# probsys/AutoGP.jl

Hardware: AMD Instinct MI355X
Metric: particle_logpdf_evals_per_sec (higher is better)
Workload: dtype f64

## Files before the change

### autogp.jl_amd/csrc/agp_chol_kernel.hpp

```cpp
#pragma once
#include <type_traits>
#include "agp_common.hpp"
#include "agp_cov_kernel.hpp"

namespace agp {

__device__ __forceinline__ double readlane_d(double v, int lane) {
  int lo = __double2loint(v), hi = __double2hiint(v);
  lo = __builtin_amdgcn_readlane(lo, lane);
  hi = __builtin_amdgcn_readlane(hi, lane);
  return __hiloint2double(hi, lo);
}

__device__ __forceinline__ d4 mfma(double a, double b, d4 c) {
  return __builtin_amdgcn_mfma_f64_16x16x4f64(a, b, c, 0, 0, 0);
}

__device__ __forceinline__ int blk_idx(int rb, int cb) { return rb * (rb + 1) / 2 + cb; }
__device__ __forceinline__ int tri_idx(int i, int j) { return i * (i + 1) / 2 + j; }

__device__ __forceinline__ void mfma_prio_on() { __builtin_amdgcn_s_setprio(1); }
__device__ __forceinline__ void mfma_prio_off() { __builtin_amdgcn_s_setprio(0); }
__device__ __forceinline__ int sblk_idx(int jb, int lb) { return jb * (jb - 1) / 2 + lb; }

// ... 139 lines not shown
    if (jb == 0) AGP_DPROBE(5);

    {
      const int nrem = NSB - 1 - jb;
      const int npair = nrem * (nrem + 1) / 2;
      auto upd = [&](int ib, int cb, bool on, d4& x) {
        (void)on;
        const double* blk = sm + blk_idx(ib, cb) * 256;
#pragma unroll
        for (int r = 0; r < 4; ++r) x[r] = blk[64 * r + l];
      };
      if (w == 0) {
        if (npair > 0) {
          double* blk = sm + blk_idx(jb + 1, jb + 1) * 256;
          const double* la = sm + blk_idx(jb + 1, jb) * 256;
          d4 x;
          double f[4];
#pragma unroll
          for (int r = 0; r < 4; ++r) { x[r] = blk[64 * r + l]; f[r] = la[64 * r + l]; }
#pragma unroll
          for (int s4 = 0; s4 < 4; ++s4) x = mfma(-f[s4], f[s4], x);
#pragma unroll
          for (int r = 0; r < 4; ++r) blk[64 * r + l] = x[r];
        }
      } else {
        int e = w, ii = 1, cc = w - 1;
        if (cc > ii) { cc -= ii + 1; ++ii; }
        auto advance = [&](int& e_, int& ii_, int& cc_) {
          e_ += 3; cc_ += 3;
          while (cc_ > ii_) { cc_ -= ii_ + 1; ++ii_; }
        };
        while (e < npair) {
          int eb[3], ib3[3], cb3[3];
#pragma unroll
          for (int u = 0; u < 3; ++u) {
            eb[u] = e; ib3[u] = jb + 1 + ii; cb3[u] = jb + 1 + cc;
            advance(e, ii, cc);
          }
          d4 x[3];
          double fa[3][4], fb[3][4];
#pragma unroll
          for (int u = 0; u < 3; ++u) {
            const bool on = eb[u] < npair;
            const int ib = on ? ib3[u] : jb + 1, cb = on ? cb3[u] : jb + 1;
            upd(ib, cb, on, x[u]);
            const double* la = sm + blk_idx(cb, jb) * 256;
            const double* lb = sm + blk_idx(ib, jb) * 256;
#pragma unroll
            for (int s4 = 0; s4 < 4; ++s4) { fa[u][s4] = -la[64 * s4 + l]; fb[u][s4] = lb[64 * s4 + l]; }
          }
#pragma unroll
          for (int s4 = 0; s4 < 4; ++s4)
#pragma unroll
            for (int u = 0; u < 3; ++u) x[u] = mfma(fa[u][s4], fb[u][s4], x[u]);
#pragma unroll
          for (int u = 0; u < 3; ++u)
            if (eb[u] < npair) {
              double* blk = sm + blk_idx(ib3[u], cb3[u]) * 256;
#pragma unroll
              for (int r = 0; r < 4; ++r) blk[64 * r + l] = x[u][r];
            }
        }
      }
      if (tid >= NB && tid - NB >= (jb + 1) * 16) {
        const int ti_ = tid - NB;
        const double* lb = sm + blk_idx(ti_ >> 4, jb) * 256;
        double t0 = rvec[ti_], t1 = 0.0;
#pragma unroll
        for (int q = 0; q < 16; q += 2) {
          t0 = fma(-lb[q * 16 + (ti_ & 15)], avec[jb * 16 + q], t0);
          t1 = fma(-lb[(q + 1) * 16 + (ti_ & 15)], avec[jb * 16 + q + 1], t1);
        }
        rvec[ti_] = t0 + t1;
      }
      if (jb == 0) AGP_DPROBE(6);
      if (w == 0 && jb + 1 < nbk) factor16(jb + 1);
      if (jb == 0) AGP_DPROBE(7);
    }
    __syncthreads();
    if (jb == 0) AGP_DPROBE(8);
  }
  if (nbk < NSB) {
    for (int jb = nbk + w; jb < NSB; jb += 4) {
      double* Wg = a.W + (((long long)p * a.wsteps + a.k % a.wsteps) * NSB + jb) * 256;
#pragma unroll
      for (int r = 0; r < 4; ++r) Wg[l15 * 16 + 4 * r + lq] = (l15 == 4 * r + lq) ? 1.0 : 0.0;
    }
    if (tid >= nbk * 16 && tid < NB) avec[tid] = 0.0;
    __syncthreads();
  }
  AGP_DPROBE(9);

  if (mark && tid == 0) *mark = (long long)wall_clock64();
  for (int bi = 0; bi < NSB * NSB / 2; ++bi) {
    const int rb = 2 * (bi >> 3) + ((tid >> 3) & 1), cb = bi & 7;
    const int c = tid >> 4, r2 = 2 * (tid & 7);
    if (rb >= cb)
      *reinterpret_cast<d2*>(Tt + (cb * 16 + c) * NB + rb * 16 + r2) = *reinterpret_cast<const d2*>(sm + blk_idx(rb, cb) * 256 + c * 16 + r2);
  }
  AGP_DPROBE(10);
  if (tid < NB) {
    vecp[tk * NB + tid] = avec[tid];
    const double dii = sm[blk_idx(tid >> 4, tid >> 4) * 256 + 17 * (tid & 15)];
    Wl[tid] = 2.0 * log(dii);
  }
  __syncthreads();
  if (w == 0) {
    double ss = avec[l] * avec[l] + avec[l + 64] * avec[l + 64];
    double ld = Wl[l] + Wl[l + 64];
#pragma unroll
    for (int off = 32; off > 0; off >>= 1) { ss += __shfl_xor(ss, off); ld += __shfl_xor(ld, off); }
    if (l == 0) {
      double* pp = a.partial + ((long long)p * (a.ntp ? a.ntp : a.nt) + tk) * 2;
      pp[0] = ld;
      pp[1] = ss;
      if (bad != 0 && a.info[p] == 0) a.info[p] = bad;
    }
  }
  if (INTRSM) {
    asm volatile("s_waitcnt vmcnt(0)" ::: "memory");
    __syncthreads();
    if (tid == 0) {
      __builtin_amdgcn_fence(__ATOMIC_RELEASE, "agent");
      asm volatile("s_waitcnt vmcnt(0)" ::: "memory");
      __hip_atomic_store(a.ready + p, a.k + 1, __ATOMIC_RELAXED, __HIP_MEMORY_SCOPE_AGENT);
      if (a.tflag != nullptr) __hip_atomic_store(a.tflag + (long long)p * a.ntri + tri_idx(tk, tk), 1, __ATOMIC_RELAXED, __HIP_MEMORY_SCOPE_AGENT);
    }
  }
  AGP_DPROBE(11);
}

__device__ __forceinline__ d2 ld_pair(const double* T, int col, int rowA) {
  return *reinterpret_cast<const d2*>(T + col * NB + rowA);
}
__device__ __forceinline__ void st_pair(double* T, int col, int rowA, double a0, double a1) {
  d2 v; v.x = a0; v.y = a1;
  *reinterpret_cast<d2*>(T + col * NB + rowA) = v;
}

struct FlowProbe { double wait; long long ph[4]; };
#ifdef AGP_EXPERIMENTS
#define AGP_TRACE(a) ((a).trace)
#else
#define AGP_TRACE(a) (static_cast<long long*>(nullptr))
#endif
#define AGP_PROBE(i) do { if (AGP_TRACE(a) && wait_acc && tid == 0) wait_acc->ph[i] = (long long)wall_clock64(); } while (0)
typedef int v4i_t __attribute__((ext_vector_type(4)));
__device__ __forceinline__ __amdgpu_buffer_rsrc_t tile_row_rsrc(const double* base) {
  return __builtin_amdgcn_make_buffer_rsrc(const_cast<double*>(base), 0, 0x7fffffff, 0x00020000);
}
__device__ __forceinline__ d2 buf_load_d2(__amdgpu_buffer_rsrc_t r, unsigned voff_bytes, int soff_bytes) {
  return __builtin_bit_cast(d2, __builtin_amdgcn_raw_buffer_load_b128(r, voff_bytes, soff_bytes, 0));
}
__device__ __forceinline__ bool flow_wait(const int* flag) {
  int spins = 0;
  while (__hip_atomic_load(flag, __ATOMIC_RELAXED, __HIP_MEMORY_SCOPE_AGENT) == 0) {
    __builtin_amdgcn_s_sleep(1);
    if (++spins > (1 << 24)) return false;
  }
  return true;
}
template <bool FACTOR, int DCOV, bool INTRSM, int DM, int GM, bool FLOW>
__device__ __forceinline__ void chol_tile(const CholArgs& a, const int p_, const int ps_, const int ti_, const int tk_,
                                          const int jmax_, const bool is_diag, double* sm, const int tid,
                                          FlowProbe* wait_acc = nullptr) {
  constexpr bool TAB = GM == 1, LAGM = GM == 2;
  const int p = __builtin_amdgcn_readfirstlane(p_), ps = __builtin_amdgcn_readfirstlane(ps_);
  const int ti = __builtin_amdgcn_readfirstlane(ti_), tk = __builtin_amdgcn_readfirstlane(tk_);
  const int jmax = __builtin_amdgcn_readfirstlane(jmax_);
  double* rvec = sm + U_MAIN_DOUBLES;
  double* avec = rvec + 128;
  double* xv = avec + 128;
  double* Wl = xv + 64;
  (void)p;
  const int l = tid & 63;
  const int w = tid >> 6;
  const int l15 = l & 15, lq = l >> 4;
  const int row0 = 32 * w + 2 * l15;
  const int row1 = row0 + 1;

  double* __restrict__ Ap = a.A + (long long)ps * a.strideA;
  double* vecp = a.vec + (long long)ps * a.ldv;

  double* __restrict__ Tt = Ap + tile_off(ti, tk);
  d4 acc[NSB][2];
  const bool prebuilt = (DCOV == 0) || (p >= a.n_fused);
  auto run_eval = [&]() {
    const ProgHdr h = a.hdr[p];
    double* tpt = sm;
    double* sig = sm + 256;
    const double* lagt = sig + h.n_cp * 256;
    const bool rankt = LAGM && a.lagr != nullptr;
    const int lstride = rankt ? a.lag_stride : 256;
    int* xrk = reinterpret_cast<int*>(sig + h.n_cp * 256 + (LAGM ? h.n_lag * lstride : 0));
    const int* rk = rankt ? xrk : nullptr;
    const bool cltm = rankt && a.clt.B != nullptr;
    int* cbl = xrk + 256;
    const int* cbp = cltm ? cbl - (a.clt.W > 0 && ti > tk ? (ti - tk) * NB - (NB - 1) : 0) : nullptr;
    double* prm = reinterpret_cast<double*>(xrk) + (rankt ? 128 + (cltm ? a.clt.nB / 2 : 0) : 0);
    int* ops = reinterpret_cast<int*>(prm + h.n_prm + 2);
    for (int i = tid; i < h.n_prm + 2; i += 256) prm[i] = a.prm[h.prm_off + i];
    for (int i = tid; i < h.n_ops; i += 256) ops[i] = (int)a.ops[h.op_off + i];
    double* etab = sm + U_MAIN_DOUBLES;
    if (AGP_EXP_TABLE && !LAGM && tid < AGP_EXP_TAB_N) etab[tid] = fm::c_exp_tab[tid];
    cov_prologue<LAGM>(a.tt, a.code, ti, tk, h, ops, prm, tpt, sig, tid, a.lagtab, a.nt, LAGM ? a.lagr : nullptr, lstride, xrk, true, a.clt, cbl);
    const double noise = !FACTOR ? 0.0 : DM == 2 ? a.noise[p] : diag_noise(a.noise, a.noise_q, p, tk, a.n1_pad);
    const bool use_tab = TAB && (h.flags & 1) != 0;
    const double* __restrict__ ltile = a.logdt + tile_off(ti, tk);
    double ltn[4] = {0.0, 0.0, 0.0, 0.0};
    auto fetch_lt = [&](int t) {
      const int cbn = t >> 1, rsn = (t & 1) ? row1 : row0;
#pragma unroll
      for (int r = 0; r < 4; ++r) ltn[r] = ltile[(cbn * 16 + 4 * r + lq) * NB + rsn];
    };
    if (use_tab) fetch_lt(0);
    const bool one_node = h.n_ops == 1;
    const int op1 = one_node ? __builtin_amdgcn_readfirstlane(ops[0]) : -1;
    const double q0 = one_node ? prm[0] : 0.0, q1 = one_node ? prm[1] : 0.0, q2 = one_node ? prm[2] : 0.0;
    const bool pure_lag = LAGM && one_node && op1 == OP_LAG && ti != tk && (ti + 1) * NB <= a.n1 && (tk + 1) * NB <= a.n1;
    if (pure_lag) {
      const double* lq_ = lagt + (NB - 1);
      const int rk0 = rk ? rk[row0] : 0, rk1 = rk ? rk[row1] : 0;
#pragma unroll
      for (int cb = 0; cb < NSB; ++cb)
#pragma unroll
        for (int r = 0; r < 4; ++r) {
          const int cs = cb * 16 + 4 * r + lq;
          double v0, v1;
          if (cbp) {
            const int rc = rk[NB + cs], e0 = rk0 - rc, e1 = rk1 - rc, d0 = e0 < 0 ? -e0 : e0, d1 = e1 < 0 ? -e1 : e1;
            v0 = -lagt[(d0 & CLT_MASK) + cbp[d0 >> CLT_SHIFT]]; v1 = -lagt[(d1 & CLT_MASK) + cbp[d1 >> CLT_SHIFT]];
          } else if (rk) {
            const int rc = rk[NB + cs], d0 = rk0 - rc, d1 = rk1 - rc;
            v0 = -lagt[d0 < 0 ? -d0 : d0]; v1 = -lagt[d1 < 0 ? -d1 : d1];
          } else {
            v0 = -lq_[row0 - cs]; v1 = -lq_[row1 - cs];
          }
          acc[cb][0][r] = v0; acc[cb][1][r] = v1;
        }
    }
    const bool pure_lin = one_node && op1 == OP_LIN && ti != tk && (ti + 1) * NB <= a.n1 && (tk + 1) * NB <= a.n1;
    if (pure_lin) {
      const double u0 = tpt[row0] - q0, u1 = tpt[row1] - q0;
#pragma unroll
      for (int cb = 0; cb < NSB; ++cb)
#pragma unroll
        for (int r = 0; r < 4; ++r) {
          const double tcc = tpt[NB + cb * 16 + 4 * r + lq] - q0;
          const double v0 = -(q1 + q2 * (u0 * tcc)), v1 = -(q1 + q2 * (u1 * tcc));
          acc[cb][0][r] = v0; acc[cb][1][r] = v1;
        }
    }
#pragma unroll 1
    for (int t = (pure_lag || pure_lin) ? 16 : 0; t < 16; ++t) {
      const int cb = t >> 1, st = t & 1;
      const int rslot = st ? row1 : row0;
      double tr[4], tc[4], out[4];
      double lt[4];
      int ri[4], ci[4];
#pragma unroll
      for (int r = 0; r < 4; ++r) lt[r] = ltn[r];
      if (use_tab && t + 1 < 16) fetch_lt(t + 1);
#pragma unroll
      for (int r = 0; r < 4; ++r) {
        const int cslot = cb * 16 + 4 * r + lq;
        tr[r] = tpt[rslot]; tc[r] = tpt[NB + cslot];
        ri[r] = rslot; ci[r] = NB + cslot;
      }
      if (one_node) {
        eval_leaf<4, (LAGM ? 3 : TAB ? 2 : 1)>(op1, q0, q1, q2, sig, lagt, tr, tc, ri, ci, lt, etab, out, rk, cbp);
      } else {
        eval_program<(DCOV > 0 ? DCOV : 4), 4, (LAGM ? 3 : TAB ? 2 : 1)>(h, ops, prm, sig, tr, tc, ri, ci, lt, out, etab, lagt, rk, lstride, cbp);
      }
      d4 v;
#pragma unroll
      for (int r = 0; r < 4; ++r)
        v[r] = -cov_finalize(out[r], ti * NB + rslot, tk * NB + cb * 16 + 4 * r + lq, a.n1, a.n1_pad, a.m2, noise);
      auto put = [&](d4& dst) { dst = v; };
      switch (t) {
        case 0: put(acc[0][0]); break;  case 1: put(acc[0][1]); break;  case 2: put(acc[1][0]); break;  case 3: put(acc[1][1]); break;
        case 4: put(acc[2][0]); break;  case 5: put(acc[2][1]); break;  case 6: put(acc[3][0]); break;  case 7: put(acc[3][1]); break;
        case 8: put(acc[4][0]); break;  case 9: put(acc[4][1]); break;  case 10: put(acc[5][0]); break; case 11: put(acc[5][1]); break;
        case 12: put(acc[6][0]); break; case 13: put(acc[6][1]); break; case 14: put(acc[7][0]); break; default: put(acc[7][1]); break;
      }
    }
    __syncthreads();
  };
  if (!prebuilt) {
    run_eval();
  } else {
#pragma unroll
    for (int cb = 0; cb < NSB; ++cb) { acc[cb][0] = d4{0.0, 0.0, 0.0, 0.0}; acc[cb][1] = d4{0.0, 0.0, 0.0, 0.0}; }
  }

  double rv = 0.0;
  if (is_diag && tid < NB) rv = vecp[tk * NB + tid];
  if (FLOW) AGP_PROBE(0);

  constexpr int KS = KB;
  constexpr int NU = KS / 4;
  constexpr int SLABS_PER_TILE = NB / KS;
  constexpr int SLAB_DOUBLES = KS * LDS_STRIDE;
  static_assert(4 * SLAB_DOUBLES <= U_MAIN_DOUBLES, "slab buffers");
  const int jfirst = FACTOR ? 0 : a.j0;
  const int nslab = (jmax - jfirst) * SLABS_PER_TILE;
  if (nslab > 0) {
    const int scol0 = tid >> 6;
    const int srow = 2 * (tid & 63);
    const unsigned offB = (unsigned)(scol0 * NB + srow);
    const unsigned offA = (unsigned)(lq * NB + row0);
    double rx = 0.0;
    const __amdgpu_buffer_rsrc_t rsA = tile_row_rsrc(Ap + tile_off(ti, 0)), rsB = tile_row_rsrc(Ap + tile_off(tk, 0));
    auto gload = [&](int s, d2 (&ra_)[NU], d2 (&rb_)[NU]) {
      const int sb = (jfirst * SLABS_PER_TILE + s) * (KS * NB * 8);
#pragma unroll
      for (int u = 0; u < NU; ++u) {
        ra_[u] = buf_load_d2(rsA, offA * 8, sb + u * (4 * NB * 8));
        rb_[u] = buf_load_d2(rsB, offB * 8, sb + u * (4 * NB * 8));
      }
      if (is_diag && tid < KS) rx = vecp[(jfirst * SLABS_PER_TILE + s) * KS + tid];
    };
    auto lstore = [&](int buf, const d2 (&ra_)[NU], const d2 (&rb_)[NU]) {
      double* Bs = sm + buf * SLAB_DOUBLES;
#pragma unroll
      for (int u = 0; u < NU; ++u) {
        *reinterpret_cast<d2*>(Bs + (scol0 + 4 * u) * LDS_STRIDE + srow) = rb_[u];
      }
      if (is_diag && tid < KS) xv[buf * KS + tid] = rx;
    };

    auto flow_ready = [&](int j) {
      const long long tw0 = AGP_TRACE(a) ? (long long)wall_clock64() : 0;
      const int* tf = a.tflag + (long long)ps * a.ntri;
      bool ok = flow_wait(tf + tri_idx(tk, j));
      if (!is_diag) ok = flow_wait(tf + tri_idx(ti, j)) && ok;
      if (!ok) a.info[ps] = -7;
      __builtin_amdgcn_fence(__ATOMIC_ACQUIRE, "agent");
      if (AGP_TRACE(a) && wait_acc) wait_acc->wait += (double)((long long)wall_clock64() - tw0);
    };
    int all_ready = 0;
    if (FLOW) {
      int probe = 0;
      if (tid == 0) {
        const int* tf = a.tflag + (long long)ps * a.ntri;
        const int jl = jfirst + (nslab - 1) / SLABS_PER_TILE;
        probe = __hip_atomic_load(tf + tri_idx(tk, jl), __ATOMIC_RELAXED, __HIP_MEMORY_SCOPE_AGENT) != 0 &&
                (is_diag || __hip_atomic_load(tf + tri_idx(ti, jl), __ATOMIC_RELAXED, __HIP_MEMORY_SCOPE_AGENT) != 0);
        if (probe) __builtin_amdgcn_fence(__ATOMIC_ACQUIRE, "agent");
        else flow_ready(jfirst);
      }
      all_ready = __syncthreads_or(probe);
    }
    d2 fx[NU], fy[NU], rb[NU];
    gload(0, fx, rb);
    lstore(0, fx, rb);
    __syncthreads();
    auto slab = [&](const int s, const int buf, const d2 (&fr)[NU], d2 (&rn)[NU], auto last) {
      constexpr bool LAST = decltype(last)::value;
      if constexpr (!LAST) gload(s + 1, rn, rb);
      const double* Bs = sm + buf * SLAB_DOUBLES;
      mfma_prio_on();
#pragma unroll
      for (int kk = 0; kk < KS / 4; ++kk) {
        const int krow = (kk * 4 + lq) * LDS_STRIDE;
        double fa[NSB];
#pragma unroll
        for (int cb = 0; cb < NSB; ++cb) fa[cb] = Bs[krow + cb * 16 + l15];
        d2 fb;
        fb = fr[kk];
#pragma unroll
        for (int cb = 0; cb < NSB; ++cb) {
          acc[cb][0] = mfma(fa[cb], fb.x, acc[cb][0]);
          acc[cb][1] = mfma(fa[cb], fb.y, acc[cb][1]);
        }
      }
      mfma_prio_off();
      if (is_diag && tid < NB) {
        const double* xs_ = xv + buf * KS;
#pragma unroll
        for (int kk = 0; kk < KS; ++kk) rv = fma(-Bs[kk * LDS_STRIDE + tid], xs_[kk], rv);
      }
      if constexpr (!LAST) lstore(buf ^ 1, rn, rb);
      if (FLOW && !all_ready && tid == 0 && s + 2 < nslab && (s + 2) % SLABS_PER_TILE == 0) flow_ready(jfirst + (s + 2) / SLABS_PER_TILE);
      __syncthreads();
    };
    constexpr std::false_type more{};
    int s = 0;
    for (; s + 2 < nslab; s += 2) {
      slab(s, 0, fx, fy, more);
      slab(s + 1, 1, fy, fx, more);
    }
    slab(s, 0, fx, fy, more);
    slab(s + 1, 1, fy, fx, std::true_type{});
  }

  if (FLOW) AGP_PROBE(1);
  if (prebuilt) {
#pragma unroll
    for (int cb = 0; cb < NSB; ++cb) {
#pragma unroll
      for (int r = 0; r < 4; ++r) {
        const d2 t2 = ld_pair(Tt, cb * 16 + 4 * r + lq, row0);
        acc[cb][0][r] -= t2.x;
        acc[cb][1][r] -= t2.y;
      }
      __builtin_amdgcn_sched_barrier(0);
    }
  }

  if (!FACTOR || (!is_diag && !INTRSM)) {
#pragma unroll
    for (int cb = 0; cb < NSB; ++cb) {
#pragma unroll
      for (int r = 0; r < 4; ++r) {
        st_pair(Tt, cb * 16 + 4 * r + lq, row0, -acc[cb][0][r], -acc[cb][1][r]);
      }
      __builtin_amdgcn_sched_barrier(0);
    }
    if (is_diag && tid < NB) vecp[tk * NB + tid] = rv;
    return;
  }

  if (!is_diag) {
    if (tid == 0) {
      if (FLOW) {
        const long long tw0 = AGP_TRACE(a) ? (long long)wall_clock64() : 0;
        if (!flow_wait(a.tflag + (long long)ps * a.ntri + tri_idx(tk, tk))) a.info[ps] = -7;
        if (AGP_TRACE(a) && wait_acc) wait_acc->wait += (double)((long long)wall_clock64() - tw0);
      } else {
        const int want = a.k + 1;
        int spins = 0;
        while (__hip_atomic_load(a.ready + ps, __ATOMIC_RELAXED, __HIP_MEMORY_SCOPE_AGENT) < want) {
          __builtin_amdgcn_s_sleep(8);
          if (++spins > (1 << 22)) { a.info[ps] = -7; break; }
        }
      }
      __builtin_amdgcn_fence(__ATOMIC_ACQUIRE, "agent");
    }
    __syncthreads();
    {
      const double* __restrict__ Lkk = Ap + tile_off(a.k, a.k);
      const double* __restrict__ Wg = a.W + ((long long)ps * a.wsteps + a.k % a.wsteps) * NSB * 256;
      const int c = tid >> 4, r = tid & 15;
#pragma unroll
      for (int jb = 1; jb < NSB; ++jb)
#pragma unroll
        for (int lb = 0; lb < jb; ++lb)
          sm[sblk_idx(jb, lb) * 256 + tid] = Lkk[(lb * 16 + c) * NB + jb * 16 + r];
#pragma unroll
      for (int u = 0; u < NSB; ++u) sm[(T_NBLK + u) * 256 + tid] = -Wg[u * 256 + tid];
    }
    __syncthreads();
    if (FLOW) AGP_PROBE(2);
#pragma unroll
    for (int jb = 0; jb < NSB; ++jb) {
#pragma unroll
      for (int lb = 0; lb < jb; ++lb) {
        const double* blk = sm + sblk_idx(jb, lb) * 256;
#pragma unroll
        for (int s4 = 0; s4 < 4; ++s4) {
          const double fl = blk[64 * s4 + l];
          acc[jb][0] = mfma(fl, acc[lb][0][s4], acc[jb][0]);
          acc[jb][1] = mfma(fl, acc[lb][1][s4], acc[jb][1]);
        }
      }
      d4 x0 = d4{0.0, 0.0, 0.0, 0.0}, x1 = d4{0.0, 0.0, 0.0, 0.0};
#pragma unroll
      for (int s4 = 0; s4 < 4; ++s4) {
        const double fw = sm[(T_NBLK + jb) * 256 + 64 * s4 + l];
        x0 = mfma(fw, acc[jb][0][s4], x0);
        x1 = mfma(fw, acc[jb][1][s4], x1);
      }
      acc[jb][0] = x0;
      acc[jb][1] = x1;
#pragma unroll
      for (int r = 0; r < 4; ++r) {
        st_pair(Tt, jb * 16 + 4 * r + lq, row0, x0[r], x1[r]);
      }
    }
    if (FLOW) {
      AGP_PROBE(3);
      asm volatile("s_waitcnt vmcnt(0)" ::: "memory");
      __syncthreads();
      if (tid == 0) {
        __builtin_amdgcn_fence(__ATOMIC_RELEASE, "agent");
        asm volatile("s_waitcnt vmcnt(0)" ::: "memory");
        __hip_atomic_store(a.tflag + (long long)ps * a.ntri + tri_idx(ti, tk), 1, __ATOMIC_RELAXED, __HIP_MEMORY_SCOPE_AGENT);
      }
    }
    return;
  }

#pragma unroll
  for (int st = 0; st < 2; ++st) {
    const int rw = st ? row1 : row0;
    const int rb = rw >> 4, rr = rw & 15;
#pragma unroll
    for (int cb = 0; cb < NSB; ++cb)
      if (rb >= cb) {
        double* blk = sm + blk_idx(rb, cb) * 256;
#pragma unroll
        for (int r = 0; r < 4; ++r) blk[(4 * r + lq) * 16 + rr] = -acc[cb][st][r];
      }
  }
  factor_diag_tile<INTRSM>(a, ps, tk, Tt, vecp, sm, rvec, avec, Wl, rv, tid);
}

template <bool FACTOR, int DCOV, bool INTRSM, int DM = 0, int GM = 0>
__global__ __launch_bounds__(256, 2) void k_chol_update(CholArgs a) {
  static_assert(GM == 0 || DCOV > 0, "the log|dt| table / the lag tables only matter to instantiations that evaluate tiles");
  static_assert(DM == 0 || (FACTOR && INTRSM), "split launches exist for the in-kernel-solve factorisation only");
  static_assert(DM == 0 || DM == 2, "the diagonal-only launch is k_chol_diag");
  __shared__ __attribute__((aligned(16))) double sm[U_MAIN_DOUBLES + U_EXTRA_DOUBLES];

  int b = blockIdx.x;
  int xcd, qq;
  int T, ti, tk, jmax;
  int pl, tl;
  if (DM == 2) {
    T = a.tiles;
    xcd = b & 7; qq = b >> 3;
    pl = qq / T; tl = a.t0 + (qq - pl * T);
    tk = a.k; ti = a.k + tl; jmax = a.k;
  } else if (FACTOR) {
    T = a.tiles;
    const int ndiag = 8 * ((a.P + 7) / 8);
    if (b < ndiag) {
      xcd = b & 7; pl = b >> 3; tl = 0;
    } else {
      b -= ndiag;
      xcd = b & 7; qq = b >> 3;
      pl = qq / (T - 1); tl = 1 + (qq - pl * (T - 1));
    }
    tk = a.k; ti = a.k + tl; jmax = a.rl ? 0 : a.k;
  } else {
    xcd = b & 7; qq = b >> 3;
    const int nt2 = a.nt - a.nt1;
    if (a.schur_diag_only) {
      T = nt2;
      pl = qq / T; tl = qq - pl * T;
      ti = tk = a.nt1 + tl; jmax = a.nt1;
    } else {
      T = nt2 * (nt2 + 1) / 2;
      pl = qq / T; tl = qq - pl * T;
      int ii = (int)((sqrt(8.0 * (double)tl + 1.0) - 1.0) * 0.5);
      while (ii * (ii + 1) / 2 > tl) --ii;
      while ((ii + 1) * (ii + 2) / 2 <= tl) ++ii;
      const int kk = tl - ii * (ii + 1) / 2;
      ti = a.nt1 + ii; tk = a.nt1 + kk; jmax = a.nt1;
    }
  }
  const int p = pl * 8 + xcd;
  if (p >= a.P) return;
  if (FACTOR && a.i0 != nullptr && ti < a.i0[p]) return;
  const int ps = (FACTOR && a.slot != nullptr) ? a.slot[p] : p;
  const bool is_diag = (DM == 2) ? false : (ti == tk);

  chol_tile<FACTOR, DCOV, INTRSM, DM, GM, false>(a, p, ps, ti, tk, jmax, is_diag, sm, threadIdx.x);
}

template <int DCOV, int GM, bool FLOW>
__device__ __forceinline__ void chol_diag_tile(const CholArgs& a, const int p_, const int ps_, const int tk_, double* sm, const int tid,
                                               FlowProbe* wait_acc = nullptr) {
  constexpr bool TAB = GM == 1, LAGM = GM == 2;
  const int p = __builtin_amdgcn_readfirstlane(p_), ps = __builtin_amdgcn_readfirstlane(ps_);
  const int tk = __builtin_amdgcn_readfirstlane(tk_);
  double* rvec = sm + U_MAIN_DOUBLES;
  double* avec = rvec + 128;
  double* xv = avec + 128;
  double* Wl = xv + 64;
  constexpr int NE = NSB + 1;
  AGP_DPROBE(0);
  const int jfirst = 0;
  const int jmax = a.rl ? 0 : a.k;
  const int l = tid & 63, w = tid >> 6, l15 = l & 15, lq = l >> 4;
  const int wu = __builtin_amdgcn_readfirstlane(w);
  const int row0 = 16 * w + l15, row1 = 16 * (NSB - 1 - w) + l15;
  int cbe[NE];
  bool st1[NE];
#pragma unroll
  for (int e = 0; e < NE; ++e) { st1[e] = e > wu; cbe[e] = st1[e] ? e - (wu + 1) : e; }

  double* __restrict__ Ap = a.A + (long long)ps * a.strideA;
  double* vecp = a.vec + (long long)ps * a.ldv;
  double* __restrict__ Tt = Ap + tile_off(tk, tk);
  d4 acc[NE];
  const bool prebuilt = (DCOV == 0) || (p >= a.n_fused);
  if (!prebuilt) {
    const ProgHdr h = a.hdr[p];
    double* tpt = sm;
    double* sig = sm + 256;
    const double* lagt = sig + h.n_cp * 256;
    const bool rankt = LAGM && a.lagr != nullptr;
    const int lstride = rankt ? a.lag_stride : 256;
    int* xrk = reinterpret_cast<int*>(sig + h.n_cp * 256 + (LAGM ? h.n_lag * lstride : 0));
    const int* rk = rankt ? xrk : nullptr;
    const bool cltm = rankt && a.clt.B != nullptr;
    int* cbl = xrk + 256;
    const int* cbp = cltm ? cbl : nullptr;
    double* prm = reinterpret_cast<double*>(xrk) + (rankt ? 128 + (cltm ? a.clt.nB / 2 : 0) : 0);
    int* ops = reinterpret_cast<int*>(prm + h.n_prm + 2);
    for (int i = tid; i < h.n_prm + 2; i += 256) prm[i] = a.prm[h.prm_off + i];
    for (int i = tid; i < h.n_ops; i += 256) ops[i] = (int)a.ops[h.op_off + i];
    double* etab = rvec;
    if (AGP_EXP_TABLE && !LAGM && tid < AGP_EXP_TAB_N) etab[tid] = fm::c_exp_tab[tid];
    cov_prologue<LAGM>(a.tt, a.code, tk, tk, h, ops, prm, tpt, sig, tid, a.lagtab, a.nt, LAGM ? a.lagr : nullptr, lstride, xrk, true, a.clt, cbl);
    const double noise = diag_noise(a.noise, a.noise_q, p, tk, a.n1_pad);
    const bool use_tab = TAB && (h.flags & 1) != 0;
    const double* __restrict__ ltile = a.logdt + tile_off(tk, tk);
    double ltn[4] = {0.0, 0.0, 0.0, 0.0};
    auto fetch_lt = [&](int e) {
      const bool s1n = e > wu;
      const int cbn = s1n ? e - (wu + 1) : e, rsn = s1n ? row1 : row0;
#pragma unroll
      for (int r = 0; r < 4; ++r) ltn[r] = ltile[(cbn * 16 + 4 * r + lq) * NB + rsn];
    };
    if (use_tab) fetch_lt(0);
    const bool one_node = h.n_ops == 1;
    const int op1 = one_node ? __builtin_amdgcn_readfirstlane(ops[0]) : -1;
    const double q0 = one_node ? prm[0] : 0.0, q1 = one_node ? prm[1] : 0.0, q2 = one_node ? prm[2] : 0.0;
    const bool full = (tk + 1) * NB <= a.n1;
    const bool pure_lag = LAGM && one_node && op1 == OP_LAG && full;
    const bool pure_lin = one_node && op1 == OP_LIN && full;
    if (pure_lag || pure_lin) {
      const double* lq_ = lagt + (NB - 1);
      const double u0 = tpt[row0] - q0, u1 = tpt[row1] - q0;
#pragma unroll
      for (int e = 0; e < NE; ++e) {
        const int rs = st1[e] ? row1 : row0;
        const double ue = st1[e] ? u1 : u0;
#pragma unroll
        for (int r = 0; r < 4; ++r) {
          const int cs = cbe[e] * 16 + 4 * r + lq;
          double v;
          if (pure_lag) {
            if (cbp) { const int d0 = rk[rs] - rk[NB + cs], d = d0 < 0 ? -d0 : d0; v = lagt[(d & CLT_MASK) + cbp[d >> CLT_SHIFT]]; }
            else if (rk) { const int d = rk[rs] - rk[NB + cs]; v = lagt[d < 0 ? -d : d]; }
            else v = lq_[rs - cs];
          } else {
            v = q1 + q2 * (ue * (tpt[NB + cs] - q0));
          }
          acc[e][r] = -(rs == cs ? v + noise : v);
        }
      }
    }
#pragma unroll 1
    for (int e = (pure_lag || pure_lin) ? NE : 0; e < NE; ++e) {
      const bool s1 = e > wu;
      const int cb = s1 ? e - (wu + 1) : e;
      const int rslot = s1 ? row1 : row0;
      double tr[4], tc[4], out[4];
      double lt[4];
      int ri[4], ci[4];
#pragma unroll
      for (int r = 0; r < 4; ++r) lt[r] = ltn[r];
      if (use_tab && e + 1 < NE) fetch_lt(e + 1);
#pragma unroll
      for (int r = 0; r < 4; ++r) {
        const int cslot = cb * 16 + 4 * r + lq;
        tr[r] = tpt[rslot]; tc[r] = tpt[NB + cslot];
        ri[r] = rslot; ci[r] = NB + cslot;
      }
      if (one_node) {
        eval_leaf<4, (LAGM ? 3 : TAB ? 2 : 1)>(op1, q0, q1, q2, sig, lagt, tr, tc, ri, ci, lt, etab, out, rk, cbp);
      } else {
        eval_program<(DCOV > 0 ? DCOV : 4), 4, (LAGM ? 3 : TAB ? 2 : 1)>(h, ops, prm, sig, tr, tc, ri, ci, lt, out, etab, lagt, rk, lstride, cbp);
      }
      d4 v;
#pragma unroll
      for (int r = 0; r < 4; ++r)
        v[r] = -cov_finalize(out[r], tk * NB + rslot, tk * NB + cb * 16 + 4 * r + lq, a.n1, a.n1_pad, a.m2, noise);
      switch (e) {
        case 0: acc[0] = v; break; case 1: acc[1] = v; break; case 2: acc[2] = v; break;
        case 3: acc[3] = v; break; case 4: acc[4] = v; break; case 5: acc[5] = v; break;
        case 6: acc[6] = v; break; case 7: acc[7] = v; break; default: acc[8] = v; break;
      }
    }
    __syncthreads();
  } else {
#pragma unroll
    for (int e = 0; e < NE; ++e) acc[e] = d4{0.0, 0.0, 0.0, 0.0};
  }

  double rv = 0.0;
  if (tid < NB) rv = vecp[tk * NB + tid];
  if (FLOW) AGP_PROBE(0);

  constexpr int KS = 2 * KB;
  constexpr int NU = KS / 4;
  constexpr int SLABS_PER_TILE = NB / KS;
  constexpr int SLAB_DOUBLES = KS * LDS_STRIDE;
  static_assert(2 * SLAB_DOUBLES <= U_MAIN_DOUBLES, "slab buffers");
  const int nslab = (jmax - jfirst) * SLABS_PER_TILE;
  if (nslab > 0) {
    const int scol0 = tid >> 6, srow = 2 * (tid & 63);
    const unsigned offB = (unsigned)(scol0 * NB + srow);
    d2 rb[NU];
    double rx = 0.0;
    const __amdgpu_buffer_rsrc_t rsB = tile_row_rsrc(Ap + tile_off(tk, 0));
    auto gload = [&](int s) {
      const int sb = (jfirst * SLABS_PER_TILE + s) * (KS * NB * 8);
#pragma unroll
      for (int u = 0; u < NU; ++u) rb[u] = buf_load_d2(rsB, offB * 8, sb + u * (4 * NB * 8));
      if (tid < KS) rx = vecp[(jfirst * SLABS_PER_TILE + s) * KS + tid];
    };
    auto lstore = [&](int buf) {
      double* Bs = sm + buf * SLAB_DOUBLES;
#pragma unroll
      for (int u = 0; u < NU; ++u) *reinterpret_cast<d2*>(Bs + (scol0 + 4 * u) * LDS_STRIDE + srow) = rb[u];
      if (tid < KS) xv[buf * KS + tid] = rx;
    };
    int fao[NE];
#pragma unroll
    for (int e = 0; e < NE; ++e) fao[e] = lq * LDS_STRIDE + cbe[e] * 16 + l15;
    const int fb0 = lq * LDS_STRIDE + row0, fb1 = lq * LDS_STRIDE + row1;
    int fbo[4];
#pragma unroll
    for (int e = 0; e < 4; ++e) fbo[e] = st1[e] ? fb1 : fb0;

    d2 rb2[NU];
    double rx2 = 0.0;
    auto gload2 = [&](int s) {
      const int sb = (jfirst * SLABS_PER_TILE + s) * (KS * NB * 8);
#pragma unroll
      for (int u = 0; u < NU; ++u) rb2[u] = buf_load_d2(rsB, offB * 8, sb + u * (4 * NB * 8));
      if (tid < KS) rx2 = vecp[(jfirst * SLABS_PER_TILE + s) * KS + tid];
    };
    auto lstore2 = [&](int buf) {
      double* Bs = sm + buf * SLAB_DOUBLES;
#pragma unroll
      for (int u = 0; u < NU; ++u) *reinterpret_cast<d2*>(Bs + (scol0 + 4 * u) * LDS_STRIDE + srow) = rb2[u];
      if (tid < KS) xv[buf * KS + tid] = rx2;
    };
    auto slab = [&](int buf) {
      const double* Bs = sm + buf * SLAB_DOUBLES;
      mfma_prio_on();
#pragma unroll
      for (int kk = 0; kk < KS / 4; ++kk) {
        const double* Bk = Bs + kk * 4 * LDS_STRIDE;
        const double f0 = Bk[fb0], f1 = Bk[fb1];
        {
          acc[0] = mfma(Bk[fao[0]], f0, acc[0]);
#pragma unroll
          for (int e = 1; e < 4; ++e) acc[e] = mfma(Bk[fao[e]], Bk[fbo[e]], acc[e]);
#pragma unroll
          for (int e = 4; e < NE; ++e) acc[e] = mfma(Bk[fao[e]], f1, acc[e]);
        }
      }
      mfma_prio_off();
      if (tid < NB) {
        const double* xs_ = xv + buf * KS;
#pragma unroll
        for (int kk = 0; kk < KS; ++kk) rv = fma(-Bs[kk * LDS_STRIDE + tid], xs_[kk], rv);
      }
    };
    auto flow_ready = [&](int j) {
      const long long tw0 = AGP_TRACE(a) ? (long long)wall_clock64() : 0;
      if (!flow_wait(a.tflag + (long long)ps * a.ntri + tri_idx(tk, j))) a.info[ps] = -7;
      __builtin_amdgcn_fence(__ATOMIC_ACQUIRE, "agent");
      if (AGP_TRACE(a) && wait_acc) wait_acc->wait += (double)((long long)wall_clock64() - tw0);
    };
    int all_ready = 0;
    if (FLOW) {
      int probe = 0;
      if (tid == 0) {
        probe = __hip_atomic_load(a.tflag + (long long)ps * a.ntri + tri_idx(tk, jmax - 1), __ATOMIC_RELAXED, __HIP_MEMORY_SCOPE_AGENT) != 0;
        if (probe) __builtin_amdgcn_fence(__ATOMIC_ACQUIRE, "agent");
        else flow_ready(jfirst);
      }
      all_ready = __syncthreads_or(probe);
    }
    gload(0);
    lstore(0);
    gload2(1);
    __syncthreads();
    for (int s = 0; s < nslab; s += 2) {
      if (s + 2 < nslab) gload(s + 2);
      slab(0);
      lstore2(1);
      __syncthreads();
      if (s + 3 < nslab) gload2(s + 3);
      slab(1);
      if (s + 2 < nslab) lstore(0);
      if (FLOW && !all_ready && tid == 0 && s + 4 < nslab && (s + 4) % SLABS_PER_TILE == 0) flow_ready(jfirst + (s + 4) / SLABS_PER_TILE);
      __syncthreads();
    }
  }

  if (FLOW) AGP_PROBE(1);
  int te = tid;
  if constexpr (FLOW) asm volatile("" : "+v"(te));
  const int l15e = te & 15, lqe = (te & 63) >> 4;
  const int row0e = 16 * (te >> 6) + l15e, row1e = 16 * (NSB - 1 - (te >> 6)) + l15e;
  if (prebuilt) {
#pragma unroll
    for (int e = 0; e < NE; ++e) {
      const int rw = st1[e] ? row1e : row0e;
#pragma unroll
      for (int r = 0; r < 4; ++r) acc[e][r] -= Tt[(cbe[e] * 16 + 4 * r + lqe) * NB + rw];
      __builtin_amdgcn_sched_barrier(0);
    }
  }

#pragma unroll
  for (int e = 0; e < NE; ++e) {
    const int rbk = st1[e] ? NSB - 1 - wu : wu;
    double* blk = sm + blk_idx(rbk, cbe[e]) * 256;
#pragma unroll
    for (int r = 0; r < 4; ++r) blk[(4 * r + lqe) * 16 + l15e] = -acc[e][r];
  }
  if (FLOW) AGP_PROBE(2);
  AGP_DPROBE(1);
  factor_diag_tile<true>(a, ps, tk, Tt, vecp, sm, rvec, avec, Wl, rv, te, (FLOW && AGP_TRACE(a) && wait_acc) ? &wait_acc->ph[3] : nullptr);
}

template <int DCOV, int GM>
__global__ __launch_bounds__(256, 2) void k_chol_diag(CholArgs a) {
  static_assert(GM == 0 || DCOV > 0, "the log|dt| table / the lag tables only matter to instantiations that evaluate tiles");
  __shared__ __attribute__((aligned(16))) double sm[U_MAIN_DOUBLES + U_EXTRA_DOUBLES];

  const int b = blockIdx.x, xcd = b & 7, pl = b >> 3;
  const int p = pl * 8 + xcd;
  if (p >= a.P) return;
  const int tk = a.k;
  if (a.i0 != nullptr && tk < a.i0[p]) return;
  const int ps = a.slot != nullptr ? a.slot[p] : p;
  chol_diag_tile<DCOV, GM, false>(a, p, ps, tk, sm, threadIdx.x);
}

template <int DCOV, int GM>
__global__ __launch_bounds__(256, 2) void k_chol_flow(CholArgs a0) {
  static_assert(GM == 0 || DCOV > 0, "the log|dt| table / the lag tables only matter to instantiations that evaluate tiles");
  __shared__ __attribute__((aligned(16))) double sm[U_MAIN_DOUBLES + U_EXTRA_DOUBLES];
  __shared__ int s_item;
  __shared__ FlowProbe s_probe;
  const int xcd = blockIdx.x & 7;
  const int Pl = (a0.P - xcd + 7) / 8;
  const int nt = a0.nt;
  const int nfac = a0.nt1;
  const int total = Pl * (nfac * nt - nfac * (nfac - 1) / 2);
  for (;;) {
    __syncthreads();
    if (threadIdx.x == 0) s_item = atomicAdd(a0.qnext + xcd, 1);
    __syncthreads();
    const int item = __builtin_amdgcn_readfirstlane(s_item);
    if (item >= total) return;
    int k = 0, rem = item, pl, tl;
    while (rem >= Pl * (nt - k)) { rem -= Pl * (nt - k); ++k; }
    if (rem < Pl) { pl = rem; tl = 0; }
    else {
      rem -= Pl;
      const int T1 = nt - k - 1;
      pl = rem / T1; tl = 1 + rem - pl * T1;
    }
    const int p = pl * 8 + xcd;
    if (a0.i0 != nullptr && k + tl < a0.i0[p]) continue;
    const int ps = a0.slot != nullptr ? a0.slot[p] : p;
    CholArgs a = a0;
    a.k = k;
    const long long t_start = AGP_TRACE(a0) ? (long long)wall_clock64() : 0;
    if (AGP_TRACE(a0) && threadIdx.x == 0) { s_probe.wait = 0.0; s_probe.ph[0] = s_probe.ph[1] = s_probe.ph[2] = s_probe.ph[3] = 0; }
    int tid = threadIdx.x;
    asm volatile("" : "+v"(tid));
    if (tl == 0) chol_diag_tile<DCOV, GM, true>(a, p, ps, k, sm, tid, &s_probe);
    else chol_tile<true, DCOV, true, 2, GM, true>(a, p, ps, k + tl, k, k, false, sm, tid, &s_probe);
    if (AGP_TRACE(a0) && threadIdx.x == 0) {
      long long gi = item;
      for (int x = 0; x < xcd; ++x) gi += ((a0.P - x + 7) / 8) * (nfac * nt - nfac * (nfac - 1) / 2);
      long long* r = AGP_TRACE(a0) + 8 * gi;
      r[0] = t_start; r[1] = (long long)wall_clock64();
      r[2] = (long long)s_probe.wait;
      r[4] = s_probe.ph[0]; r[5] = s_probe.ph[1]; r[6] = s_probe.ph[2]; r[7] = s_probe.ph[3];
      r[3] = ((long long)blockIdx.x << 48) | ((long long)(tl == 0 ? 0 : 1) << 44) | ((long long)p << 24) | ((long long)(k + tl) << 12) | k;
    }
  }
}

#ifdef AGP_KERNEL_TU_MAIN
__global__ __launch_bounds__(256, 2) void k_chol_trsm(CholArgs a) {
  __shared__ __attribute__((aligned(16))) double ls[T_LDS_DOUBLES];
  const int b = blockIdx.x;
  const int xcd = b & 7, qq = b >> 3;
  const int T = a.nt - a.k - 1;
  const int pl = qq / T, tl = qq - pl * T;
  const int p = pl * 8 + xcd;
  if (p >= a.P) return;
  const int ti = a.k + 1 + tl;

  const int tid = threadIdx.x;
  const int l = tid & 63, w = tid >> 6;
  const int l15 = l & 15, lq = l >> 4;

  double* __restrict__ Ap = a.A + (long long)p * a.strideA;
  const double* __restrict__ Lkk = Ap + tile_off(a.k, a.k);
  double* __restrict__ Tt = Ap + tile_off(ti, a.k);
  const double* __restrict__ Wg = a.W + ((long long)p * a.wsteps + a.k % a.wsteps) * NSB * 256;

  {
    const int c = tid >> 4, r = tid & 15;
#pragma unroll
    for (int jb = 1; jb < NSB; ++jb)
#pragma unroll
      for (int lb = 0; lb < jb; ++lb)
        ls[sblk_idx(jb, lb) * 256 + tid] = -Lkk[(lb * 16 + c) * NB + jb * 16 + r];
    double* lw = ls + T_NBLK * 256;
#pragma unroll
    for (int u = 0; u < NSB; ++u) lw[u * 256 + tid] = Wg[u * 256 + tid];
  }
  d4 X[2][NSB];
  d4 nxt[2];
#pragma unroll
  for (int st = 0; st < 2; ++st)
#pragma unroll
    for (int r = 0; r < 4; ++r) nxt[st][r] = Tt[(4 * r + lq) * NB + (2 * w + st) * 16 + l15];
  __syncthreads();
  const double* lw = ls + T_NBLK * 256;

#pragma unroll
  for (int jb = 0; jb < NSB; ++jb) {
    d4 acc[2] = {nxt[0], nxt[1]};
    if (jb + 1 < NSB) {
#pragma unroll
      for (int st = 0; st < 2; ++st)
#pragma unroll
        for (int r = 0; r < 4; ++r)
          nxt[st][r] = Tt[((jb + 1) * 16 + 4 * r + lq) * NB + (2 * w + st) * 16 + l15];
    }
#pragma unroll
    for (int lb = 0; lb < jb; ++lb) {
      const double* blk = ls + sblk_idx(jb, lb) * 256;
#pragma unroll
      for (int s4 = 0; s4 < 4; ++s4) {
        const double fl = blk[64 * s4 + l];
        acc[0] = mfma(fl, X[0][lb][s4], acc[0]);
        acc[1] = mfma(fl, X[1][lb][s4], acc[1]);
      }
    }
    d4 x0 = d4{0.0, 0.0, 0.0, 0.0}, x1 = d4{0.0, 0.0, 0.0, 0.0};
// ... 287 lines not shown
```

Baseline: 20570.

## Interleave triangular-solve vector FMAs with MFMA loop and peel slab pipeline branches

Moves the per-slab rv dot-product update (forward substitution on the right-hand vector) out of a separate tail loop restricted to threads below NB and interleaves it with the MFMA accumulation, so the scalar FMAs overlap with matrix-core work. All threads now compute rv on a masked row index. The vector slab load becomes an unconditional buffer load, and the non-FLOW slab loop is peeled so the last iteration drops its branches. In the FLOW path, boundary loads and stores now run unconditionally on clamped indices, which adds redundant memory traffic and extra register and LDS pressure.

Measured after the change: 20690, median of 6. No clear change (+0.6%).

```diff
diff --git a/autogp.jl_amd/csrc/agp_chol_kernel.hpp b/autogp.jl_amd/csrc/agp_chol_kernel.hpp
--- a/autogp.jl_amd/csrc/agp_chol_kernel.hpp
+++ b/autogp.jl_amd/csrc/agp_chol_kernel.hpp
@@ -315,6 +315,9 @@
 __device__ __forceinline__ d2 buf_load_d2(__amdgpu_buffer_rsrc_t r, unsigned voff_bytes, int soff_bytes) {
   return __builtin_bit_cast(d2, __builtin_amdgcn_raw_buffer_load_b128(r, voff_bytes, soff_bytes, 0));
 }
+__device__ __forceinline__ double buf_load_d1(__amdgpu_buffer_rsrc_t r, unsigned voff_bytes, int soff_bytes) {
+  return __builtin_bit_cast(double, __builtin_amdgcn_raw_buffer_load_b64(r, voff_bytes, soff_bytes, 0));
+}
 __device__ __forceinline__ bool flow_wait(const int* flag) {
   int spins = 0;
   while (__hip_atomic_load(flag, __ATOMIC_RELAXED, __HIP_MEMORY_SCOPE_AGENT) == 0) {
@@ -518,43 +521,63 @@
     gload(0, fx, rb);
     lstore(0, fx, rb);
     __syncthreads();
-    auto slab = [&](const int s, const int buf, const d2 (&fr)[NU], d2 (&rn)[NU], auto last) {
+    const int rrow = tid & (NB - 1);
+    auto slab = [&](const int s, const int buf, const d2 (&fr)[NU], d2 (&rn)[NU], auto last, auto diag) {
       constexpr bool LAST = decltype(last)::value;
+      constexpr bool DIAG = decltype(diag)::value;
       if constexpr (!LAST) gload(s + 1, rn, rb);
       const double* Bs = sm + buf * SLAB_DOUBLES;
+      const double* xs_ = xv + buf * KS;
       mfma_prio_on();
 #pragma unroll
       for (int kk = 0; kk < KS / 4; ++kk) {
         const int krow = (kk * 4 + lq) * LDS_STRIDE;
         double fa[NSB];
-#pragma unroll
-        for (int cb = 0; cb < NSB; ++cb) fa[cb] = Bs[krow + cb * 16 + l15];
+        if constexpr (!DIAG) {
+#pragma unroll
+          for (int cb = 0; cb < NSB; ++cb) fa[cb] = Bs[krow + cb * 16 + l15];
+        }
         d2 fb;
         fb = fr[kk];
 #pragma unroll
-        for (int cb = 0; cb < NSB; ++cb) {
-          acc[cb][0] = mfma(fa[cb], fb.x, acc[cb][0]);
-          acc[cb][1] = mfma(fa[cb], fb.y, acc[cb][1]);
+        for (int h = 0; h < 2; ++h) {
+          if constexpr (DIAG) {
+#pragma unroll
+            for (int cb = h * (NSB / 2); cb < (h + 1) * (NSB / 2); ++cb) fa[cb] = Bs[krow + cb * 16 + l15];
+          }
+#pragma unroll
+          for (int cb = h * (NSB / 2); cb < (h + 1) * (NSB / 2); ++cb) {
+            acc[cb][0] = mfma(fa[cb], fb.x, acc[cb][0]);
+            acc[cb][1] = mfma(fa[cb], fb.y, acc[cb][1]);
+          }
+          if constexpr (DIAG) {
+            const double* Bc = Bs + (kk * 4 + 2 * h) * LDS_STRIDE + rrow;
+            const d2 x2 = *reinterpret_cast<const d2*>(xs_ + 4 * kk + 2 * h);
+            rv = fma(-Bc[0], readlane_d(x2.x, 0), rv);
+            rv = fma(-Bc[LDS_STRIDE], readlane_d(x2.y, 0), rv);
+            asm volatile("" : "+v"(rv));
+            __builtin_amdgcn_sched_barrier(0);
+          }
         }
       }
       mfma_prio_off();
-      if (is_diag && tid < NB) {
-        const double* xs_ = xv + buf * KS;
-#pragma unroll
-        for (int kk = 0; kk < KS; ++kk) rv = fma(-Bs[kk * LDS_STRIDE + tid], xs_[kk], rv);
-      }
       if constexpr (!LAST) lstore(buf ^ 1, rn, rb);
       if (FLOW && !all_ready && tid == 0 && s + 2 < nslab && (s + 2) % SLABS_PER_TILE == 0) flow_ready(jfirst + (s + 2) / SLABS_PER_TILE);
       __syncthreads();
     };
-    constexpr std::false_type more{};
-    int s = 0;
-    for (; s + 2 < nslab; s += 2) {
-      slab(s, 0, fx, fy, more);
-      slab(s + 1, 1, fy, fx, more);
-    }
-    slab(s, 0, fx, fy, more);
-    slab(s + 1, 1, fy, fx, std::true_type{});
+    auto slabs = [&](auto diag) {
+      constexpr std::false_type more{};
+      int s = 0;
+      for (; s + 2 < nslab; s += 2) {
+        slab(s, 0, fx, fy, more, diag);
+        slab(s + 1, 1, fy, fx, more, diag);
+      }
+      slab(s, 0, fx, fy, more, diag);
+      slab(s + 1, 1, fy, fx, std::true_type{}, diag);
+    };
+    if constexpr (DM == 2) slabs(std::false_type{});
+    else if (is_diag) slabs(std::true_type{});
+    else slabs(std::false_type{});
   }
 
   if (FLOW) AGP_PROBE(1);
@@ -861,11 +884,14 @@
     d2 rb[NU];
     double rx = 0.0;
     const __amdgpu_buffer_rsrc_t rsB = tile_row_rsrc(Ap + tile_off(tk, 0));
+    const __amdgpu_buffer_rsrc_t rsV = tile_row_rsrc(vecp);
+    const unsigned offV = (unsigned)((tid & (KS - 1)) * 8);
+    auto vload = [&](int s) { return buf_load_d1(rsV, offV, (jfirst * SLABS_PER_TILE + s) * (KS * 8)); };
     auto gload = [&](int s) {
       const int sb = (jfirst * SLABS_PER_TILE + s) * (KS * NB * 8);
 #pragma unroll
       for (int u = 0; u < NU; ++u) rb[u] = buf_load_d2(rsB, offB * 8, sb + u * (4 * NB * 8));
-      if (tid < KS) rx = vecp[(jfirst * SLABS_PER_TILE + s) * KS + tid];
+      rx = vload(s);
     };
     auto lstore = [&](int buf) {
       double* Bs = sm + buf * SLAB_DOUBLES;
@@ -887,7 +913,7 @@
       const int sb = (jfirst * SLABS_PER_TILE + s) * (KS * NB * 8);
 #pragma unroll
       for (int u = 0; u < NU; ++u) rb2[u] = buf_load_d2(rsB, offB * 8, sb + u * (4 * NB * 8));
-      if (tid < KS) rx2 = vecp[(jfirst * SLABS_PER_TILE + s) * KS + tid];
+      rx2 = vload(s);
     };
     auto lstore2 = [&](int buf) {
       double* Bs = sm + buf * SLAB_DOUBLES;
@@ -895,27 +921,37 @@
       for (int u = 0; u < NU; ++u) *reinterpret_cast<d2*>(Bs + (scol0 + 4 * u) * LDS_STRIDE + srow) = rb2[u];
       if (tid < KS) xv[buf * KS + tid] = rx2;
     };
+    const int rrow = tid & (NB - 1);
     auto slab = [&](int buf) {
       const double* Bs = sm + buf * SLAB_DOUBLES;
+      const double* xs_ = xv + buf * KS;
       mfma_prio_on();
 #pragma unroll
       for (int kk = 0; kk < KS / 4; ++kk) {
         const double* Bk = Bs + kk * 4 * LDS_STRIDE;
+        double fa[NE], fm[4], cl[4];
         const double f0 = Bk[fb0], f1 = Bk[fb1];
-        {
-          acc[0] = mfma(Bk[fao[0]], f0, acc[0]);
-#pragma unroll
-          for (int e = 1; e < 4; ++e) acc[e] = mfma(Bk[fao[e]], Bk[fbo[e]], acc[e]);
-#pragma unroll
-          for (int e = 4; e < NE; ++e) acc[e] = mfma(Bk[fao[e]], f1, acc[e]);
-        }
+#pragma unroll
+        for (int e = 0; e < NE; ++e) fa[e] = Bk[fao[e]];
+#pragma unroll
+        for (int e = 1; e < 4; ++e) fm[e] = Bk[fbo[e]];
+#pragma unroll
+        for (int c = 0; c < 4; ++c) cl[c] = Bk[c * LDS_STRIDE + rrow];
+        const d2 x01 = *reinterpret_cast<const d2*>(xs_ + 4 * kk), x23 = *reinterpret_cast<const d2*>(xs_ + 4 * kk + 2);
+        __builtin_amdgcn_sched_barrier(0);
+        acc[0] = mfma(fa[0], f0, acc[0]);
+#pragma unroll
+        for (int e = 1; e < 4; ++e) acc[e] = mfma(fa[e], fm[e], acc[e]);
+#pragma unroll
+        for (int e = 4; e < NE; ++e) acc[e] = mfma(fa[e], f1, acc[e]);
+        rv = fma(-cl[0], x01.x, rv);
+        rv = fma(-cl[1], x01.y, rv);
+        rv = fma(-cl[2], x23.x, rv);
+        rv = fma(-cl[3], x23.y, rv);
+        asm volatile("" : "+v"(rv));
+        __builtin_amdgcn_sched_barrier(0);
       }
       mfma_prio_off();
-      if (tid < NB) {
-        const double* xs_ = xv + buf * KS;
-#pragma unroll
-        for (int kk = 0; kk < KS; ++kk) rv = fma(-Bs[kk * LDS_STRIDE + tid], xs_[kk], rv);
-      }
     };
     auto flow_ready = [&](int j) {
       const long long tw0 = AGP_TRACE(a) ? (long long)wall_clock64() : 0;
@@ -937,16 +973,33 @@
     lstore(0);
     gload2(1);
     __syncthreads();
-    for (int s = 0; s < nslab; s += 2) {
-      if (s + 2 < nslab) gload(s + 2);
-      slab(0);
-      lstore2(1);
-      __syncthreads();
-      if (s + 3 < nslab) gload2(s + 3);
-      slab(1);
-      if (s + 2 < nslab) lstore(0);
-      if (FLOW && !all_ready && tid == 0 && s + 4 < nslab && (s + 4) % SLABS_PER_TILE == 0) flow_ready(jfirst + (s + 4) / SLABS_PER_TILE);
-      __syncthreads();
+    if constexpr (!FLOW) {
+      auto pair = [&](const int s, auto last) {
+        constexpr bool LAST = decltype(last)::value;
+        if constexpr (!LAST) gload(s + 2);
+        slab(0);
+        lstore2(1);
+        __syncthreads();
+        if constexpr (!LAST) gload2(s + 3);
+        slab(1);
+        if constexpr (!LAST) lstore(0);
+        __syncthreads();
+      };
+      int s = 0;
+      for (; s + 2 < nslab; s += 2) pair(s, std::false_type{});
+      pair(s, std::true_type{});
+    } else {
+      for (int s = 0; s < nslab; s += 2) {
+        gload(s + 2 < nslab ? s + 2 : s);
+        slab(0);
+        lstore2(1);
+        __syncthreads();
+        gload2(s + 3 < nslab ? s + 3 : s + 1);
+        slab(1);
+        lstore(0);
+        if (!all_ready && tid == 0 && s + 4 < nslab && (s + 4) % SLABS_PER_TILE == 0) flow_ready(jfirst + (s + 4) / SLABS_PER_TILE);
+        __syncthreads();
+      }
     }
   }
 
```
